# Chemical118/TREW

Hardware: AMD Instinct MI355X
Metric: Gbases/s scanned (short 5 32, 150 bp reads) (higher is better)
Workload: dtype u32

## Files before the change

### include/trew_hip.h

```cpp
#ifndef TREW_HIP_H
#define TREW_HIP_H

#include <stddef.h>
#include <stdint.h>

#ifdef __cplusplus
extern "C" {
#endif

#define TREW_HIP_ABI_VERSION 4

enum {
    TREW_MODE_SHORT = 0,
    TREW_MODE_PAIR = 1,
    TREW_MODE_LONG = 2,
    TREW_MODE_SEGMENT = 3
};

enum {
    TREW_TABLE_FORWARD_HIGH = 0,
    TREW_TABLE_FORWARD_LOW = 1,
    TREW_TABLE_BACKWARD_HIGH = 2,
    TREW_TABLE_BACKWARD_LOW = 3,
    TREW_TABLE_BOTH_HIGH = 4,
// ... 58 lines not shown
typedef struct {
    int32_t k;
    int32_t table;
    uint64_t word_lo;
    uint64_t word_hi;
    uint64_t count;
} trew_hip_row;

typedef struct trew_hip_ctx trew_hip_ctx;

int trew_hip_init(const trew_hip_params *params, trew_hip_ctx **out);
void trew_hip_destroy(trew_hip_ctx *ctx);
const char *trew_hip_last_error(const trew_hip_ctx *ctx);

int trew_hip_submit(trew_hip_ctx *ctx, const trew_hip_batch *batch, int slot);
int trew_hip_submit_ascii(trew_hip_ctx *ctx, const trew_hip_ascii_batch *batch, int slot);
int trew_hip_pack_ascii(trew_hip_ctx *ctx, const trew_hip_ascii_batch *batch, uint32_t *words, uint64_t words_cap, uint64_t *n_words);
int trew_hip_wait(trew_hip_ctx *ctx, int slot);

int trew_hip_collect(trew_hip_ctx *ctx, int table, trew_hip_row *rows, uint64_t cap, uint64_t *n_rows);
int trew_hip_reset_tables(trew_hip_ctx *ctx);
int trew_hip_add_rows(trew_hip_ctx *ctx, const trew_hip_row *rows, uint64_t n_rows);

int trew_hip_collect_device(trew_hip_ctx *ctx, trew_hip_row *d_rows, uint64_t cap, uint64_t *n_rows);
int trew_hip_add_rows_device(trew_hip_ctx *ctx, const trew_hip_row *d_rows, uint64_t n_rows);
int trew_hip_merge(trew_hip_ctx *dst, trew_hip_ctx *src);
int trew_hip_add_gathered_device(trew_hip_ctx *ctx, const trew_hip_row *d_buf, uint32_t n_slices, uint32_t own_slice,
                                 uint64_t slice_rows, void *producer_stream, uint64_t *max_rows);
int trew_hip_collect_slice_device(trew_hip_ctx *ctx, trew_hip_row *d_slice, uint64_t slice_rows, void *consumer_stream, uint64_t *n_rows);

int trew_hip_table_pressure(trew_hip_ctx *ctx, uint64_t *used_slots, uint64_t *total_slots, uint64_t *spilled_rows,
                            uint64_t *spill_capacity);

#define TREW_DEBUG_COUNTERS 8
int trew_hip_debug_counters(trew_hip_ctx *ctx, uint64_t *out, int n);

int trew_hip_debug_worklist(trew_hip_ctx *ctx, int slot, uint32_t *units, uint64_t cap, uint64_t *n);

int trew_hip_segment_results(trew_hip_ctx *ctx, int slot, int32_t *k_high, int32_t *k_low,
                             uint64_t *seq_high, uint64_t *seq_low, uint64_t *seq_high_hi, uint64_t *seq_low_hi,
                             uint64_t n_reads);
int trew_hip_filter_masks(trew_hip_ctx *ctx, const trew_hip_batch *batch, uint64_t *cand, int slots_per_read);

int trew_hip_last_timing(trew_hip_ctx *ctx, int slot, float *ms_filter, float *ms_exact, uint64_t *n_flagged);

typedef struct {
    int32_t k;
    int32_t reserved;
    uint64_t word;
} trew_hip_motif;
typedef struct {
    uint32_t windows_fwd, windows_rev, tract_start_fwd, tract_len_fwd, tract_start_rev, tract_len_rev;
} trew_hip_annot;
#define TREW_ANNOT_MAX_MOTIFS 8

int trew_motif_parse(const char *text, trew_hip_motif *out);
int trew_hip_annotate(trew_hip_ctx *ctx, const trew_hip_batch *batch, int slot, const trew_hip_motif *motifs, int n_motifs);
int trew_hip_annotate_results(trew_hip_ctx *ctx, int slot, trew_hip_annot *out, uint64_t cap, uint64_t *n, float *ms_kernel);
int trew_annotate_host(const uint32_t *words, const uint32_t *offsets, const uint32_t *lengths, uint64_t n_reads,
                       const trew_hip_motif *motifs, int n_motifs, trew_hip_annot *out);

typedef struct {
    uint32_t covered_fwd, head_len_fwd, head_cov_fwd, tail_len_fwd, tail_cov_fwd;
    uint32_t covered_rev, head_len_rev, head_cov_rev, tail_len_rev, tail_cov_rev;
} trew_hip_tract;
int trew_hip_tracts(trew_hip_ctx *ctx, const trew_hip_batch *batch, int slot, const trew_hip_motif *motifs, int n_motifs, int penalty);
int trew_hip_tracts_results(trew_hip_ctx *ctx, int slot, trew_hip_tract *out, uint64_t cap, uint64_t *n, float *ms_kernel);
// ... 61 lines not shown
```

### trew_amd/capi.py

```python
from __future__ import annotations

import ctypes as C
import os

import numpy as np

_HERE = os.path.dirname(os.path.abspath(__file__))
LIB_PATH = os.environ.get("TREW_HIP_LIB") or os.path.join(_HERE, "lib", "libtrew_hip.so")

MODE_SHORT, MODE_PAIR, MODE_LONG, MODE_SEGMENT = 0, 1, 2, 3
FLAG_NO_FILTER = 1
FLAG_DEBUG_POISON_LDS = 32
FLAG_NO_TIMING = 64
FLAG_COMPAT_G1 = 512
FLAG_TRACK_PRESSURE = 256
FLAG_DEBUG_NO_JOINT = 2048
FLAG_DEBUG_NO_UNI_DRAIN = 4096
FLAG_DEBUG_NO_GROUP = 1024
FLAG_DEBUG_ANNOT_GENERAL = 8192
FLAG_DEBUG_WIDE_NO_WAIT = 128
TABLE_NAMES = ("forward_high", "forward_low", "backward_high", "backward_low", "both_high", "both_low")

EXPORTED_SYMBOLS = (
    "trew_hip_init", "trew_hip_destroy", "trew_hip_last_error", "trew_hip_submit", "trew_hip_wait",
    "trew_hip_collect", "trew_hip_reset_tables", "trew_hip_add_rows", "trew_hip_segment_results",
    "trew_hip_filter_masks", "trew_hip_last_timing", "trew_pack_words", "trew_pack_reads",
    "trew_synth_short_ascii", "trew_synth_short_device", "trew_synth_pair_ascii", "trew_synth_pair_device",
    "trew_hip_malloc", "trew_hip_free", "trew_hip_memcpy_h2d", "trew_hip_memcpy_d2h", "trew_hip_abi_version",
    "trew_pack_pairs", "trew_hip_host_alloc", "trew_hip_host_free", "trew_hip_device_count",
    "trew_synth_long_lengths", "trew_synth_long_ascii", "trew_synth_long_device",
    "trew_hip_collect_device", "trew_hip_add_rows_device", "trew_hip_merge", "trew_hip_table_pressure",
    "trew_hip_add_gathered_device", "trew_hip_collect_slice_device", "trew_hip_debug_counters", "trew_hip_debug_worklist", "trew_hip_submit_ascii", "trew_hip_pack_ascii",
    "trew_motif_parse", "trew_hip_annotate", "trew_hip_annotate_results", "trew_annotate_host",
    "trew_hip_tracts", "trew_hip_tracts_results", "trew_tracts_host",
    "trew_hip_intervals", "trew_hip_intervals_results", "trew_intervals_host",
    "trew_hip_variants", "trew_hip_variants_results", "trew_variants_host",
)
DEBUG_COUNTERS = ("strict_rerun", "windows_fallback", "wide_spin_timeout", "inserted", "inserted_wide", "group_punt", "group_routed", "group_target")


class Params(C.Structure):
    _fields_ = [
        ("min_mer", C.c_int32), ("max_mer", C.c_int32),
        ("low_baseline", C.c_double), ("high_baseline", C.c_double),
        ("slice_length", C.c_int32), ("mode", C.c_int32), ("device", C.c_int32), ("n_slots", C.c_int32),
        ("max_batch_words", C.c_uint64), ("max_batch_reads", C.c_uint64),
        ("table_log2_slots", C.c_uint32), ("flags", C.c_uint32),
        ("max_batch_ascii_bytes", C.c_uint64),
    ]


class Batch(C.Structure):
    _fields_ = [
        ("words", C.c_void_p), ("n_words", C.c_uint64),
        ("offsets", C.c_void_p), ("lengths", C.c_void_p),
        ("uniform_length", C.c_uint32), ("uniform_stride", C.c_uint32),
        ("n_reads", C.c_uint64), ("on_device", C.c_int32), ("max_length", C.c_int32),
    ]


class AsciiBatch(C.Structure):
    _fields_ = [
        ("bases", C.c_void_p), ("n_bytes", C.c_uint64),
        ("byte_offsets", C.c_void_p), ("lengths", C.c_void_p), ("word_offsets", C.c_void_p),
        ("uniform_length", C.c_uint32), ("reserved", C.c_uint32), ("n_reads", C.c_uint64),
    ]


class Row(C.Structure):
    _fields_ = [("k", C.c_int32), ("table", C.c_int32), ("word_lo", C.c_uint64), ("word_hi", C.c_uint64),
                ("count", C.c_uint64)]
# ... 638 lines not shown
```

### trew_amd/csrc/kernels/prefilter.inc

```


__device__ __forceinline__ u32 xor_and(u32 x, u32 y, u32 m) { return __builtin_amdgcn_bitop3_b32(x, y, m, 0x28); }

__device__ __forceinline__ u64 all_k_mask(int kmin, int kmax) {
    if (kmax < kmin) return 0;
    u64 hi = kmax >= 64 ? ~0ull : ((1ull << kmax) - 1ull);
    u64 lo = (1ull << (kmin - 1)) - 1ull;
    return hi & ~lo;
}

template <int NW, int WS>
__device__ __forceinline__ u32 shr_word(const u32 (&x)[NW], int j, u32 bs) {
    const u32 lo = (j + WS < NW) ? x[j + WS < NW ? j + WS : 0] : 0u;
    const u32 hi = (j + WS + 1 < NW) ? x[j + WS + 1 < NW ? j + WS + 1 : 0] : 0u;
    return alignbit(hi, lo, bs);
}

template <int NW, int WS, int NWW>
__device__ __forceinline__ void filter_k(const u32 (&P1)[NW], const u32 (&P2)[NW], const u32 (&P3)[NW],
                                         const u32 (&v1)[NW], u32 (&V)[NW], int k, float lowf, u32 &cand_lo, u32 &cand_hi) {
    const u32 bs = (u32) k & 31u;
    u32 c01 = 0, c10 = 0, c11 = 0, count = 0;
#pragma unroll
    for (int j = 0; j < NWW; j++) {
// ... 281 lines not shown
            FilterRangeUni<NW, 2, NW, true>::run(P1, P2, P3, gmin > 64 ? gmin : 64, gmax, L, kmin, kmax, thr_row, dbg, vd);
        } else {
            FilterRangeUni<NW, 0, NW, false>::run(P1, P2, P3, gmin, g31, L, kmin, kmax, thr_row, false, vd);
            FilterRangeUni<NW, 1, NW, false>::run(P1, P2, P3, gmin > 32 ? gmin : 32, gmax < 63 ? gmax : 63, L, kmin, kmax, thr_row, false, vd);
            FilterRangeUni<NW, 2, NW, false>::run(P1, P2, P3, gmin > 64 ? gmin : 64, gmax, L, kmin, kmax, thr_row, false, vd);
            vd.flagm = vd.hasm;
        }
    }
}

struct HalvesP {
    u32 P1[3], P2[3];
};
__device__ __forceinline__ void halves_prefix(const u32 (&lo)[3], const u32 (&hi)[3], int L, HalvesP &o) {
    u32 none[3];
    segment_setup<3, false, false>(lo, hi,  lo, L,  none, o.P1, o.P2, none);
}
__device__ __forceinline__ u32 bcnt_acc_s(u32 x, int acc) {
    u32 d;
    asm("v_bcnt_u32_b32 %0, %1, %2" : "=v"(d) : "v"(x), "s"(acc));
    return d;
}
__device__ __forceinline__ void halves_signs(u32 F1a, u32 F2a, u32 F1b, u32 F2b, int n2, int n1, int K, u32 &x, u32 &t) {
    u32 a = bcnt_acc_s(F1a, n2);
    u32 b = bcnt_acc_s(F2a, n2);
    u32 c = bcnt_acc_s(F1a & F2a, n1);
    a = bcnt_acc(F1b, a);
    b = bcnt_acc(F2b, b);
    c = bcnt_acc(F1b & F2b, c);
    const u32 p = a - c, q = b - c;
    x = __builtin_amdgcn_bitop3_b32(p, q, c, 0x80);
    t = a + q + (u32) K;
}
__device__ __forceinline__ u64 halves_verdict(u32 xA, u32 tA, u32 xB, u32 tB) {
    const u32 y = __builtin_amdgcn_bitop3_b32(xA, xB, tA, 0x40);
    const u32 z = __builtin_amdgcn_bitop3_b32(y, tB, tB, 0x30);
    return __ballot((int) z >= 0);
}
struct Thr8 {
    int4 a, b;
};
__device__ __forceinline__ Thr8 load_thr8(const int4 *p) {
    typedef int v8i __attribute__((ext_vector_type(8)));
    typedef const __attribute__((address_space(4))) v8i *cptr;
    const v8i v = *(cptr) (unsigned long long) p;
    Thr8 o;
    o.a = make_int4(v[0], v[1], v[2], v[3]);
    o.b = make_int4(v[4], v[5], v[6], v[7]);
    return o;
}
__device__ __forceinline__ int4 load_thr4(const int4 *p) {
    typedef int v4i __attribute__((ext_vector_type(4)));
    typedef const __attribute__((address_space(4))) v4i *cptr;
    const v4i v = *(cptr) (unsigned long long) p;
    return make_int4(v.x, v.y, v.z, v.w);
}

__device__ __forceinline__ const int4 *joint_thresholds(const int2 *thr_tab) { return (const int4 *) (thr_tab + kThrRows * kThrRow); }

__device__ __forceinline__ u64 filter_halves_uni(const HalvesP &A, const HalvesP &Bh, int L, int klo, int khi, const int4 *__restrict__ thr_row,
                                                 const u32 *wm_tab) {
    u64 trig = 0;
    int k = klo;
    const int4 *tp = thr_row + (klo - 1);
    {
        int b = L - 64;
        b = b > khi ? khi : b;
        auto probe = [&](u32 bs, const int4 t) __attribute__((always_inline)) -> u64 {
            u32 xA, tA, xB, tB;
            halves_signs(A.P1[0] ^ alignbit(A.P1[1], A.P1[0], bs), A.P2[0] ^ alignbit(A.P2[1], A.P2[0], bs), A.P1[1] ^ alignbit(A.P1[2], A.P1[1], bs),
                         A.P2[1] ^ alignbit(A.P2[2], A.P2[1], bs), t.x, t.y, t.z, xA, tA);
            halves_signs(Bh.P1[0] ^ alignbit(Bh.P1[1], Bh.P1[0], bs), Bh.P2[0] ^ alignbit(Bh.P2[1], Bh.P2[0], bs), Bh.P1[1] ^ alignbit(Bh.P1[2], Bh.P1[1], bs),
                         Bh.P2[1] ^ alignbit(Bh.P2[2], Bh.P2[1], bs), t.x, t.y, t.z, xB, tB);
            return halves_verdict(xA, tA, xB, tB);
        };
        for (; k + 1 <= b; k += 2, tp += 2) {
            const Thr8 t8 = load_thr8(tp);
            trig |= probe((u32) k, t8.a);
            trig |= probe((u32) k + 1u, t8.b);
        }
        if (k <= b) {
            trig |= probe((u32) k, load_thr4(tp));
            k++, tp++;
        }
    }
    if (k <= khi) {
        const int b = khi;
        const int s = L > 63 ? L - 63 : 0;
        const u64 QA1 = container64(A.P1, s), QA2 = container64(A.P2, s), QB1 = container64(Bh.P1, s), QB2 = container64(Bh.P2, s);
        u32 sh = (u32) (k - s);
        typedef const __attribute__((address_space(3))) u32 *lds_u32;
        u32 wa = (u32) (unsigned long long) (lds_u32) wm_tab + 4u * (u32) (63 - (L - k));
        asm volatile("" : "+v"(wa));
        auto probe = [&](u32 shk, u32 wmk, const int4 t) __attribute__((always_inline)) -> u64 {
            const u64 SA1 = QA1 >> shk, SA2 = QA2 >> shk, SB1 = QB1 >> shk, SB2 = QB2 >> shk;
            const u32 gA1 = xor_and(A.P1[1], (u32) (SA1 >> 32), wmk), gA2 = xor_and(A.P2[1], (u32) (SA2 >> 32), wmk);
            const u32 gB1 = xor_and(Bh.P1[1], (u32) (SB1 >> 32), wmk), gB2 = xor_and(Bh.P2[1], (u32) (SB2 >> 32), wmk);
            u32 xA, tA, xB, tB;
            halves_signs(A.P1[0] ^ (u32) SA1, A.P2[0] ^ (u32) SA2, gA1, gA2, t.x, t.y, t.z, xA, tA);
            halves_signs(Bh.P1[0] ^ (u32) SB1, Bh.P2[0] ^ (u32) SB2, gB1, gB2, t.x, t.y, t.z, xB, tB);
            return halves_verdict(xA, tA, xB, tB);
        };
        for (; k + 1 <= b; k += 2, sh += 2u, wa += 8u, tp += 2) {
            const Thr8 t8 = load_thr8(tp);
            const u32 wm0 = *(lds_u32) (unsigned long long) wa, wm1 = *(lds_u32) (unsigned long long) (wa + 4u);
            trig |= probe(sh, wm0, t8.a);
            trig |= probe(sh + 1u, wm1, t8.b);
        }
        if (k <= b) trig |= probe(sh, *(lds_u32) (unsigned long long) wa, load_thr4(tp));
    }
    return trig;
}

constexpr int kCntThr = 97;
__device__ __forceinline__ int4 count_thresholds(int c, float lowf) {
    const float prod = __fmul_rn((float) c, lowf);
    const int ithr = (int) floorf(prod) + 1;
    return make_int4(-2 * ithr, -ithr, 4 * ithr - c - 1, ithr);
}

struct DrainHalf {
    u32 P1[3], P2[3], P3[3];
    u32 V[3];
};
__device__ __forceinline__ void drain_half_init(const u32 (&lo)[3], const u32 (&hi)[3], const u32 (&nm)[3], int L, bool active, DrainHalf &h) {
    segment_setup<3, false, true, true>(lo, hi, nm, L, h.V, h.P1, h.P2, h.P3);
#pragma unroll
    for (int j = 0; j < 3; j++) h.V[j] = active ? h.V[j] : 0u;
}
__device__ __forceinline__ void drain_v_step3(u32 (&V)[3]) {
    V[0] &= alignbit(V[1], V[0], 1u);
    V[1] &= alignbit(V[2], V[1], 1u);
    V[2] &= V[2] >> 1;
}
template <int N>
__device__ __forceinline__ int drain_signs(const u32 (&F1)[N], const u32 (&F2)[N], const int4 th) {
    u32 a = (u32) th.x, b = (u32) th.x, c = (u32) th.y;
#pragma unroll
    for (int j = 0; j < N; j++) {
        a = bcnt_acc(F1[j], a);
        b = bcnt_acc(F2[j], b);
        c = bcnt_acc(F1[j] & F2[j], c);
    }
    const u32 p = a - c, q = b - c;
    const u32 t = a + q + (u32) th.z;
    return (int) __builtin_amdgcn_bitop3_b32(__builtin_amdgcn_bitop3_b32(p, q, c, 0x80), t, t, 0x30);
}
template <int N>
__device__ __forceinline__ bool drain_pass8(const u32 (&F1)[N], const u32 (&F2)[N], const u32 (&F3)[N], const u32 (&V)[N], u32 count, int ithr) {
    const u32 m8 = max_bucket8<N>(F1, F2, F3, V, count);
    return (int) m8 >= ithr;
}

__device__ __forceinline__ bool drain_uni_applies(const DevParams &P, u32 UL, int gmax_run) {
    const int n_halves = P.mode == TREW_MODE_PAIR ? 4 : (P.mode == TREW_MODE_SHORT ? 2 : 0);
    if (n_halves == 0) return false;
    for (int slot = n_halves; slot < mode_slots(P.mode); slot++)
        if (get_segment(P.mode, slot, UL, UL, P.min_mer, P.max_mer, P.slice_len).valid) return false;
    for (int p = 0; p < n_halves; p += 2) {
        const Segment a = get_segment(P.mode, p, UL, UL, P.min_mer, P.max_mer, P.slice_len);
        const Segment b = get_segment(P.mode, p + 1, UL, UL, P.min_mer, P.max_mer, P.slice_len);
        const int la = (int) a.len, lb = (int) b.len, lmin = la < lb ? la : lb, lmax = la < lb ? lb : la;
        const int khi = a.kmax < gmax_run ? a.kmax : gmax_run;
        if (!(a.valid && b.valid && a.kmin == b.kmin && a.kmax == b.kmax && lmax <= 95 && lmax - lmin <= 1 && a.kmin >= 1 && khi <= lmin)) return false;
    }
    return true;
}

__device__ __forceinline__ bool filter_deferred_uni(const DevParams &P, const DevBatch &B, u64 unit, bool active, int gmax_run,
                                                    const int4 *cnt_thr) {
    const u32 UL = B.uniform_length;
    ReadRef rd[2];
    unit_reads(P, B, unit, active, rd);
    const u64 actm = __ballot(active);
    u64 flag = 0;
    const int n_halves = P.mode == TREW_MODE_PAIR ? 4 : 2;
    for (int p = 0; p < n_halves && flag != actm; p += 2) {
        const Segment sA = get_segment(P.mode, p, UL, UL, P.min_mer, P.max_mer, P.slice_len);
        const Segment sB = get_segment(P.mode, p + 1, UL, UL, P.min_mer, P.max_mer, P.slice_len);
        const int LA = rfl_i((int) sA.len), LB = rfl_i((int) sB.len), Lmax = LA < LB ? LB : LA;
        const int klo = rfl_i(sA.kmin > P.min_mer ? sA.kmin : P.min_mer), khi = rfl_i(sA.kmax < gmax_run ? sA.kmax : gmax_run);
        DrainHalf A, Bh;
        {
            u32 lo[3], hi[3], nm[3];
            load_planes<3>(sA.mate ? rd[1] : rd[0], sA.start, lo, hi, nm);
            drain_half_init(lo, hi, nm, LA, active, A);
            load_planes<3>(sB.mate ? rd[1] : rd[0], sB.start, lo, hi, nm);
            drain_half_init(lo, hi, nm, LB, active, Bh);
        }
        for (int t = 1; t < klo; t++) {
            drain_v_step3(A.V);
            drain_v_step3(Bh.V);
        }
        int k = klo;
        {
            const int b = khi < Lmax - 64 ? khi : Lmax - 64;
            auto half3 = [&](const DrainHalf &h, u32 bs) __attribute__((always_inline)) -> u64 {
                const u32 cnt = bcnt_acc(h.V[2], bcnt_acc(h.V[1], __popc(h.V[0])));
                const int4 th = cnt_thr[cnt];
                u32 F1[3], F2[3];
#pragma unroll
                for (int j = 0; j < 3; j++) {
                    F1[j] = xor_and(h.P1[j], alignbit(j < 2 ? h.P1[j < 2 ? j + 1 : 0] : 0u, h.P1[j], bs), h.V[j]);
                    F2[j] = xor_and(h.P2[j], alignbit(j < 2 ? h.P2[j < 2 ? j + 1 : 0] : 0u, h.P2[j], bs), h.V[j]);
                }
                const u64 p4 = __ballot(drain_signs<3>(F1, F2, th) >= 0);
                u64 p8 = 0;
                if (p4 & ~flag) {
                    u32 F3[3];
#pragma unroll
                    for (int j = 0; j < 3; j++) F3[j] = h.P3[j] ^ alignbit(j < 2 ? h.P3[j < 2 ? j + 1 : 0] : 0u, h.P3[j], bs);
                    p8 = __ballot(drain_pass8<3>(F1, F2, F3, h.V, cnt, th.w));
                }
                return p8;
            };
            for (; k <= b && flag != actm; k++) {
                flag |= half3(A, (u32) k);
                flag |= half3(Bh, (u32) k);
                drain_v_step3(A.V);
                drain_v_step3(Bh.V);
            }
        }
        if (k <= khi && flag != actm) {
            const int oA = LA > 63 ? LA - 63 : 0, oB = LB > 63 ? LB - 63 : 0;
            const u64 QA1 = container64(A.P1, oA), QA2 = container64(A.P2, oA), QB1 = container64(Bh.P1, oB), QB2 = container64(Bh.P2, oB);
            u64 VA = ((u64) A.V[1] << 32) | A.V[0], VB = ((u64) Bh.V[1] << 32) | Bh.V[0];
            auto half2 = [&](const DrainHalf &h, u64 Q1, u64 Q2, u64 V, int s) __attribute__((always_inline)) -> u64 {
                const u32 v0 = (u32) V, v1 = (u32) (V >> 32);
                const u32 cnt = bcnt_acc(v1, __popc(v0));
                const int4 th = cnt_thr[cnt];
                const u32 sh = (u32) (k - s);
                const u64 S1 = Q1 >> sh, S2 = Q2 >> sh;
                const u32 F1[2] = {xor_and(h.P1[0], (u32) S1, v0), xor_and(h.P1[1], (u32) (S1 >> 32), v1)};
                const u32 F2[2] = {xor_and(h.P2[0], (u32) S2, v0), xor_and(h.P2[1], (u32) (S2 >> 32), v1)};
                const u64 p4 = __ballot(drain_signs<2>(F1, F2, th) >= 0);
                u64 p8 = 0;
                if (p4 & ~flag) {
                    const u64 S3 = container64(h.P3, s) >> sh;
                    const u32 F3[2] = {h.P3[0] ^ (u32) S3, h.P3[1] ^ (u32) (S3 >> 32)};
                    const u32 Vw[2] = {v0, v1};
                    p8 = __ballot(drain_pass8<2>(F1, F2, F3, Vw, cnt, th.w));
                }
                return p8;
            };
            for (; k <= khi && flag != actm; k++) {
                flag |= half2(A, QA1, QA2, VA, oA);
                flag |= half2(Bh, QB1, QB2, VB, oB);
                VA &= VA >> 1;
                VB &= VB >> 1;
            }
        }
    }
    return (flag >> lane_id()) & 1ull;
}

constexpr u32 kFilterThreads = TREW_FILTER_THREADS;
constexpr u32 kStage = kFilterThreads == 256 ? 1024 : 192;
constexpr u32 kDefer = 2 * kFilterThreads;

template <int NW>
#ifndef TREW_FILTER3_WAVES
#define TREW_FILTER3_WAVES 6
#endif
#ifndef TREW_FILTER5_WAVES
#define TREW_FILTER5_WAVES 6
#endif
__global__ __launch_bounds__(kFilterThreads, (NW <= 3 ? TREW_FILTER3_WAVES : (NW == 5 ? TREW_FILTER5_WAVES : 1))) void filter_kernel(DevParams P, DevBatch B, u32 *wl, u32 *wl_count, u32 wl_cap,
                                                                u64 *dbg_masks, int dbg_slots, int max_seg, u32 *diag,
                                                                const int2 *__restrict__ thr_tab) {
#ifdef TREW_AB_FILTER_PRIO
    __builtin_amdgcn_s_setprio(TREW_AB_FILTER_PRIO);
#endif
    __shared__ u32 stage[kStage];
    __shared__ u32 stage_n, flush_base;
    __shared__ u32 defer_n;
    u32 defer_seen = 0;
    if (threadIdx.x == 0) stage_n = 0;
    __syncthreads();
    auto flush = [&]() __attribute__((always_inline)) {
        const u32 n = stage_n;
        if (n) {
            if (threadIdx.x == 0) flush_base = atomicAdd(wl_count, n);
            __syncthreads();
            const u32 fb = flush_base;
            for (u32 i = threadIdx.x; i < n; i += blockDim.x) {
                if (fb + i < wl_cap)
                    wl[fb + i] = stage[i];
                else
                    atomicAdd(&diag[kDiagWorklistDrop], 1u);
            }
            __syncthreads();
            if (threadIdx.x == 0) stage_n = 0;
        }
        __syncthreads();
    };
    auto append = [&](bool flag, u32 unit) __attribute__((always_inline)) {
        wave_append(&stage_n, flag, [&](u32 at) __attribute__((always_inline)) { stage[at] = unit; });
        __syncthreads();
        const bool full = stage_n > kStage - kFilterThreads;
        defer_seen = defer_n;
        __syncthreads();
        if (full) flush();
    };
    const int nslots = mode_slots(P.mode);
    const int gmax_run = (P.flags & TREW_FLAG_DEBUG_NO_KLOOP) ? P.min_mer - 1 : P.max_mer;
    auto general = [&](u64 unit, bool active) __attribute__((always_inline)) -> u64 {
        ReadRef rd[2];
        unit_reads(P, B, unit, active, rd);
        u64 any = 0;
#pragma unroll
        for (int slot = 0; slot < kMaxSlots; slot++) {
            if (slot < nslots) {
                u64 mask = 0;
                Segment sg = get_segment(P.mode, slot, rd[0].len, rd[1].len, P.min_mer, P.max_mer, P.slice_len);
                const bool ok = active && sg.valid && sg.len <= (u32) (32 * NW - 1);
                if (__any(ok)) {
                    u32 lo[NW], hi[NW], nm[NW];
                    const ReadRef &r = sg.mate ? rd[1] : rd[0];
                    if (ok) {
                        load_planes<NW>(r, sg.start, lo, hi, nm);
                    } else {
#pragma unroll
                        for (int j = 0; j < NW; j++) {
                            lo[j] = hi[j] = 0;
                            nm[j] = 0xffffffffu;
                        }
                    }
                    u64 m;
                    if (P.flags & TREW_FLAG_NO_FILTER)
                        m = all_k_mask(sg.kmin, sg.kmax);
                    else
                        m = filter_segment<NW>(lo, hi, nm, ok ? (int) sg.len : 0, sg.kmin, sg.kmax, P.min_mer, gmax_run, max_seg, P.lowf);
                    mask = ok ? m : 0ull;
                }
                if (active && sg.valid && sg.len > (u32) (32 * NW - 1)) mask = all_k_mask(sg.kmin, sg.kmax);
                any |= mask;
                if (dbg_masks && active && slot < dbg_slots) dbg_masks[unit * (u64) dbg_slots + slot] = mask;
            }
        }
        return any;
    };

    __shared__ u32 defer[kDefer];
    __shared__ unsigned char defer_kind[kDefer];
    __shared__ u32 wm_tab[34];
    if (threadIdx.x < 34) wm_tab[threadIdx.x] = threadIdx.x < 32 ? 0xffffffffu >> threadIdx.x : 0u;
    __shared__ int4 cnt_thr[kCntThr];
    for (u32 i = threadIdx.x; i < (u32) kCntThr; i += blockDim.x) cnt_thr[i] = count_thresholds((int) i, P.lowf);
    const u32 UL = B.uniform_length;
    const bool uni = NW <= 5 && UL != 0 && thr_tab != nullptr && P.mode != TREW_MODE_LONG && !(P.flags & TREW_FLAG_NO_FILTER);
    const bool uni_drain = NW == 3 && uni && !dbg_masks && !(P.flags & TREW_FLAG_DEBUG_NO_UNI_DRAIN) && drain_uni_applies(P, UL, gmax_run);
    if (threadIdx.x == 0) defer_n = 0;
    __syncthreads();
    __shared__ u32 next_chunk[2];
    constexpr u32 kChunkShards = 8;
    const u32 my_shard = blockIdx.x & (kChunkShards - 1u);
    auto shard_ctr = [&](u32 sh) __attribute__((always_inline)) { return wl_count + 32u + 32u * sh + kChunkCounterWord; };
    u64 chunk = blockIdx.x;
    u32 round = 0;
    for (;;) {
        const bool more = chunk * kFilterThreads < B.n_units;
        if (more) {
            const u64 unit = chunk * kFilterThreads + threadIdx.x;
            const bool active = unit < B.n_units;
            u32 nxt = 0;
            if (threadIdx.x == 0) nxt = gridDim.x + kChunkShards * atomicAdd(shard_ctr(my_shard), 1u) + my_shard;
            u64 any = 0;
            bool dfr = active, dfr_n = false;
            if constexpr (NW <= 5) {
                if (uni) {
                    ReadRef rd[2];
                    unit_reads(P, B, unit, active, rd);
                    dfr = false;
                    int slot0 = 0;
                    if constexpr (NW == 3) {
                        const int n_halves = P.mode == TREW_MODE_PAIR ? 4 : (P.mode == TREW_MODE_SHORT ? 2 : 0);
                        for (; slot0 + 1 < n_halves && !dbg_masks && !(P.flags & TREW_FLAG_DEBUG_NO_JOINT); slot0 += 2) {
                            const Segment sA = get_segment(P.mode, slot0, UL, UL, P.min_mer, P.max_mer, P.slice_len);
                            const Segment sB = get_segment(P.mode, slot0 + 1, UL, UL, P.min_mer, P.max_mer, P.slice_len);
                            const int L = rfl_i((int) sA.len);
                            const int klo = rfl_i(sA.kmin > P.min_mer ? sA.kmin : P.min_mer), khi = rfl_i(sA.kmax < gmax_run ? sA.kmax : gmax_run);
                            const bool uneq = sB.len == sA.len + 1u;
                            if (!(sA.valid && sB.valid && (sA.len == sB.len || uneq) && sA.len <= 95u && sA.kmin == sB.kmin && sA.kmax == sB.kmax &&
                                  klo >= L + 1 - kUniSubsetMax && khi <= L - 32 && klo <= 31))
                                break;
                            u32 loA[3], hiA[3], nmA[3], loB[3], hiB[3], nmB[3];
                            load_planes<3>(sA.mate ? rd[1] : rd[0], sA.start, loA, hiA, nmA);
                            load_planes<3>(sB.mate ? rd[1] : rd[0], sB.start, loB, hiB, nmB);
                            const u32 anyn = segment_has_n<3>(nmA, L) | segment_has_n<3>(nmB, (int) sB.len);
                            dfr = dfr || (active && anyn != 0);
                            dfr_n = dfr_n || (active && anyn != 0);
                            HalvesP hA, hB;
                            halves_prefix(loA, hiA, L, hA);
                            halves_prefix(loB, hiB, L, hB);
                            const u64 trig = filter_halves_uni(hA, hB, L, klo, khi, joint_thresholds(thr_tab) + (uneq ? 2 + slot0 / 2 : slot0 / 2) * kThrRow, wm_tab);
                            dfr = dfr || (active && any == 0 && ((trig >> lane_id()) & 1ull) != 0);
                        }
                    }
                    for (int slot = slot0; slot < nslots; slot++) {
                        const Segment sg = get_segment(P.mode, slot, UL, UL, P.min_mer, P.max_mer, P.slice_len);
                        if (!sg.valid) continue;
                        if (sg.len > (u32) (32 * NW - 1)) {
                            dfr = dfr || active;
                            continue;
                        }
                        u32 lo[NW], hi[NW], nm[NW];
                        const ReadRef r = sg.mate ? rd[1] : rd[0];
                        load_planes<NW>(r, sg.start, lo, hi, nm);
                        u32 anyn = 0;
#pragma unroll
                        for (int j = 0; j < NW; j++) {
                            const int bits = (int) sg.len - 32 * j;
                            const u32 lm = low_mask(bits);
                            anyn |= nm[j] & lm;
                        }
                        UniVerdict vd;
                        filter_segment_uni<NW>(lo, hi, (int) sg.len, sg.kmin, sg.kmax, P.min_mer, gmax_run, thr_tab + slot * kThrRow, dbg_masks != nullptr, vd);
                        dfr = dfr || (active && anyn != 0);
                        dfr_n = dfr_n || (active && anyn != 0);
                        any |= (vd.flagm >> lane_id()) & 1ull;
                        if (dbg_masks && active && anyn == 0 && slot < dbg_slots)
                            dbg_masks[unit * (u64) dbg_slots + slot] = ((((u64) vd.chi) << 32) | vd.clo) & all_k_mask(sg.kmin, sg.kmax);
                    }
                }
            }
            {
                wave_append(&defer_n, dfr, [=](u32 at) __attribute__((always_inline)) {
                    defer[at] = (u32) unit;
                    defer_kind[at] = dfr_n ? 1 : 0;
                });
            }
            if (threadIdx.x == 0) next_chunk[round & 1u] = nxt;
            append(active && !dfr && any != 0, (u32) unit);
            chunk = next_chunk[round & 1u];
            if (chunk * kFilterThreads >= B.n_units) {
                __syncthreads();
                if (threadIdx.x == 0) {
                    u64 c = chunk;
                    for (u32 att = 1; att < kChunkShards && c * kFilterThreads >= B.n_units; att++) {
                        const u32 sh = (my_shard + att) & (kChunkShards - 1u);
                        c = (u64) gridDim.x + (u64) kChunkShards * atomicAdd(shard_ctr(sh), 1u) + sh;
                    }
                    next_chunk[round & 1u] = (u32) (c < 0xffffffffull ? c : 0xffffffffull);
                }
                __syncthreads();
                chunk = next_chunk[round & 1u];
                __syncthreads();
            }
            round++;
        }
        const u32 dn = defer_seen;
        if (dn >= kFilterThreads || (!more && dn > 0u)) {
            const u32 take = dn < kFilterThreads ? dn : kFilterThreads;
            const u32 at = dn - take;
            const bool active2 = threadIdx.x < take;
            const u32 unit2 = active2 ? defer[at + threadIdx.x] : 0u;
            const bool n2 = active2 && defer_kind[at + threadIdx.x] != 0;
            __syncthreads();
            if (threadIdx.x == 0) defer_n = at;
#ifndef TREW_AB_SKIP_DRAIN
            const u64 any2 = uni_drain ? (u64) filter_deferred_uni(P, B, unit2, active2, gmax_run, cnt_thr) : general(unit2, active2);
#else
            u64 any2 = 0;
            u32 keep = unit2;
            asm volatile("" : "+v"(keep), "+v"(any2));
            (void) keep;
#endif
            append(active2 && any2 != 0 && !n2, unit2);
            append(active2 && any2 != 0 && n2, unit2);
        } else if (!more) {
            break;
        }
    }
    flush();
}
```

### trew_amd/csrc/trew_capi.cpp

```cpp
#include <hip/hip_runtime.h>

#include <algorithm>
#include <atomic>
#include <cmath>
#include <cstdio>
#include <cstdlib>
#include <cstring>
#include <mutex>
#include <string>
#include <thread>
#include <vector>

#include "trew_common.hpp"
#include "trew_launch.hpp"
#include "trew_measures_host.hpp"
#include "trew_synth.hpp"

using namespace trew;

namespace {

enum Measure { kAnnotate, kTracts, kIntervals, kVariants, kMeasures };
const char *const kMeasureName[kMeasures] = {"annotate", "tracts", "intervals", "variants"};
struct DevBuf {
// ... 941 lines not shown
    HIPCHK(ctx, hipMemsetAsync(ctx->d_row_flags, 0, kRowFlagWords * 4, st));
    HIPCHK(ctx, launch_add_gathered(st, ctx->table, d_buf, n_slices, own_slice, slice_rows, ctx->d_row_flags));
    u32 flags[kRowFlagWords] = {0, 0, 0, 0};
    HIPCHK(ctx, hipMemcpyAsync(flags, ctx->d_row_flags, sizeof(flags), hipMemcpyDeviceToHost, st));
    HIPCHK(ctx, hipStreamSynchronize(st));
    if (max_rows) *max_rows = ((u64) flags[kRowFlagMaxHi] << 32) | flags[kRowFlagMaxLo];
    if (flags[kRowFlagBad]) return fail(ctx, "trew_hip_add_gathered_device: row out of range (nothing was added)");
    if (flags[kRowFlagOverflow]) return 0;
    u32 diag[kDiagWords];
    return check_diag(ctx, diag);
}

extern "C" int trew_hip_debug_worklist(trew_hip_ctx *ctx, int slot, uint32_t *units, uint64_t cap, uint64_t *n) {
    if (!ctx || !n) return -1;
    if (slot < 0 || slot >= (int) ctx->slots.size()) return fail(ctx, "slot out of range");
    HIPCHK(ctx, hipSetDevice(ctx->p.device));
    Slot &s = ctx->slots[(size_t) slot];
    HIPCHK(ctx, hipStreamSynchronize(s.stream));
    u32 c = 0;
    if (s.n_launches) HIPCHK(ctx, hipMemcpy(&c, s.d_wl_count + ((s.n_launches - 1) & 1) * kWlCountWords, 4, hipMemcpyDeviceToHost));
    c = (u32) std::min<u64>(c, ctx->p.max_batch_reads);
    *n = c;
    const u64 take = std::min<u64>(c, cap);
    if (units && take) HIPCHK(ctx, hipMemcpy(units, s.d_wl, take * 4, hipMemcpyDeviceToHost));
    return 0;
}

extern "C" int trew_hip_debug_counters(trew_hip_ctx *ctx, uint64_t *out, int n) {
    if (!ctx || !out || n < 0) return -1;
    if (int rc = sync_all(ctx)) return rc;
    u32 diag[kDiagWords], fb[kFallbackWords];
    HIPCHK(ctx, hipMemcpy(diag, ctx->table.overflow, sizeof(diag), hipMemcpyDeviceToHost));
    HIPCHK(ctx, fallback_counters_read(fb));
    const u32 v[TREW_DEBUG_COUNTERS] = {fb[kFallbackStrictRerun], fb[kFallbackWindows], fb[kFallbackWideSpin], diag[kDiagInserted], diag[kDiagInsertedWide], fb[kFallbackGroupPunt], fb[kFallbackGroupRouted], fb[kFallbackGroupTarget]};
    for (int i = 0; i < n; i++) out[i] = i < TREW_DEBUG_COUNTERS ? v[i] : 0;
    return 0;
}

extern "C" int trew_hip_merge(trew_hip_ctx *dst, trew_hip_ctx *src) {
    if (!dst || !src) return -1;
    if (dst == src) return fail(dst, "trew_hip_merge: source and destination are the same context");
    std::mutex *m1 = &dst->table_mu, *m2 = &src->table_mu;
    if (m2 < m1) std::swap(m1, m2);
    std::lock_guard<std::mutex> l1(*m1), l2(*m2);
    if (int rc = sync_all(src)) return rc;
    u64 n = 0;
    if (int rc = compact_to(src, -1, nullptr, 0, &n)) return rc;
    if (n == 0) return 0;
    if (int rc = ensure_rows(src, &src->d_collect_rows, &src->collect_cap, n)) return rc;
    if (int rc = compact_to(src, -1, src->d_collect_rows, src->collect_cap, &n)) return rc;
    if (int rc = sync_all(dst)) return rc;
    if (int rc = ensure_rows(dst, &dst->d_add_rows, &dst->add_cap, n)) return rc;
    HIPCHK(dst, hipSetDevice(dst->p.device));
    HIPCHK(dst, hipMemcpyPeerAsync(dst->d_add_rows, dst->p.device, src->d_collect_rows, src->p.device, n * sizeof(trew_hip_row), dst->slots[0].stream));
    return add_device_rows_locked(dst, dst->d_add_rows, n, false);
}

extern "C" int trew_hip_segment_results(trew_hip_ctx *ctx, int slot, int32_t *k_high, int32_t *k_low,
                                        uint64_t *seq_high, uint64_t *seq_low, uint64_t *seq_high_hi, uint64_t *seq_low_hi,
                                        uint64_t n_reads) {
    if (!ctx) return -1;
    if (ctx->p.mode != TREW_MODE_SEGMENT) return fail(ctx, "segment results exist only in TREW_MODE_SEGMENT");
    if (slot < 0 || slot >= (int) ctx->slots.size()) return fail(ctx, "slot out of range");
    if (int rc = trew_hip_wait(ctx, slot)) return rc;
    Slot &s = ctx->slots[(size_t) slot];
    if (n_reads > s.n_units) return fail(ctx, "n_reads exceeds the last batch");
    if (k_high) HIPCHK(ctx, hipMemcpy(k_high, s.res.k_high, n_reads * 4, hipMemcpyDeviceToHost));
// ... 615 lines not shown
```

### trew_amd/csrc/trew_common.hpp

```cpp
#pragma once
#include <stdint.h>

#include "../../include/trew_hip.h"

namespace trew {

typedef uint32_t u32;
typedef uint64_t u64;

constexpr int kMaxSlots = 6;
constexpr int kMaxSegBases = 1023;
constexpr int kTablePartBits = 9;
constexpr int kThrRows = kMaxSlots + 2;
constexpr int kThrJointRows = 4;
constexpr int kThrRow = 66;
constexpr size_t kThrTableBytes = (size_t) kThrRows * kThrRow * 8 + (size_t) kThrJointRows * kThrRow * 16;
constexpr int kThrNever = 1 << 20;

struct DevParams {
    int min_mer, max_mer;
    double low, high;
    float lowf;
    int slice_len;
    int mode;
// ... 1 lines not shown
};

struct DevBatch {
    const u32 *words;
    const u32 *offsets;
    const u32 *lengths;
    u32 uniform_length;
    u32 uniform_stride;
    u64 n_reads;
    u64 n_units;
};

constexpr int kChunkCounterWord = 16;

enum {
    kDiagOverflow = 0,
    kDiagWorklistDrop = 1,
    kDiagIntentDrop = 2,
    kDiagInserted = 3,
    kDiagInsertedWide = 4,
    kDiagKernarg = 5,
    kDiagSpillRows = 6,
    kDiagG1Drop = 7,
    kDiagWords = 16
};

enum {
    kFallbackStrictRerun = 0,
    kFallbackWindows = 1,
    kFallbackWideSpin = 2,
    kFallbackGroupPunt = 3,
    kFallbackGroupRouted = 4,
    kFallbackGroupTarget = 5,
    kFallbackWords = 8
};

enum { kRowFlagBad = 0, kRowFlagOverflow = 1, kRowFlagMaxLo = 2, kRowFlagMaxHi = 3, kRowFlagWords = 4 };

struct DevTable {
    u64 *keys;
    u64 *counts;
    u32 log2_part_slots;
    u32 *overflow;
    const struct DevWide *wide;
};

struct DevG1 {
    trew_hip_row *log;
    u32 *counters;
    unsigned char *pair_flags;
    u32 log_cap;
};


struct DevWide {
    u64 *wtag, *wlo, *whi, *wcount;
    u32 wide_log2_slots;
    u32 spill_cap;
    trew_hip_row *spill_rows;
    u32 *spill_n;
    u32 spin_limit;
};

struct DevTableG1 {
    DevTable t;
    DevG1 g;
// ... 143 lines not shown
```

Measured before the change: 1996.

## Drain only the single flagged half when one read half passes the joint filter

The joint halves prefilter now keeps a separate pass verdict for each half instead of a combined ballot. When exactly one half of a unit needs exact checking, the unit goes to a new per-half defer list and a single-half drain that processes only that half's planes. This avoids running the two-half drain on halves the filter already rejected. The cost is an extra shared-memory defer queue, extra wave appends and an added debug atomic counter on every drain.

Result: faster. 2090 (median of 6 runs) (+4.7%).

```diff
diff --git a/include/trew_hip.h b/include/trew_hip.h
--- a/include/trew_hip.h
+++ b/include/trew_hip.h
@@ -114,7 +114,7 @@
 int trew_hip_table_pressure(trew_hip_ctx *ctx, uint64_t *used_slots, uint64_t *total_slots, uint64_t *spilled_rows,
                             uint64_t *spill_capacity);
 
-#define TREW_DEBUG_COUNTERS 8
+#define TREW_DEBUG_COUNTERS 10
 int trew_hip_debug_counters(trew_hip_ctx *ctx, uint64_t *out, int n);
 
 int trew_hip_debug_worklist(trew_hip_ctx *ctx, int slot, uint32_t *units, uint64_t cap, uint64_t *n);
diff --git a/trew_amd/capi.py b/trew_amd/capi.py
--- a/trew_amd/capi.py
+++ b/trew_amd/capi.py
@@ -36,7 +36,8 @@
     "trew_hip_intervals", "trew_hip_intervals_results", "trew_intervals_host",
     "trew_hip_variants", "trew_hip_variants_results", "trew_variants_host",
 )
-DEBUG_COUNTERS = ("strict_rerun", "windows_fallback", "wide_spin_timeout", "inserted", "inserted_wide", "group_punt", "group_routed", "group_target")
+DEBUG_COUNTERS = ("strict_rerun", "windows_fallback", "wide_spin_timeout", "inserted", "inserted_wide", "group_punt", "group_routed", "group_target",
+                  "half_drain", "unit_drain")
 
 
 class Params(C.Structure):
diff --git a/trew_amd/csrc/kernels/prefilter.inc b/trew_amd/csrc/kernels/prefilter.inc
--- a/trew_amd/csrc/kernels/prefilter.inc
+++ b/trew_amd/csrc/kernels/prefilter.inc
@@ -337,11 +337,7 @@
     x = __builtin_amdgcn_bitop3_b32(p, q, c, 0x80);
     t = a + q + (u32) K;
 }
-__device__ __forceinline__ u64 halves_verdict(u32 xA, u32 tA, u32 xB, u32 tB) {
-    const u32 y = __builtin_amdgcn_bitop3_b32(xA, xB, tA, 0x40);
-    const u32 z = __builtin_amdgcn_bitop3_b32(y, tB, tB, 0x30);
-    return __ballot((int) z >= 0);
-}
+__device__ __forceinline__ u32 halves_note(u32 acc, u32 x, u32 t) { return __builtin_amdgcn_bitop3_b32(acc, x, t, 0x40); }
 struct Thr8 {
     int4 a, b;
 };
@@ -363,29 +359,30 @@
 
 __device__ __forceinline__ const int4 *joint_thresholds(const int2 *thr_tab) { return (const int4 *) (thr_tab + kThrRows * kThrRow); }
 
-__device__ __forceinline__ u64 filter_halves_uni(const HalvesP &A, const HalvesP &Bh, int L, int klo, int khi, const int4 *__restrict__ thr_row,
-                                                 const u32 *wm_tab) {
-    u64 trig = 0;
+__device__ __forceinline__ void filter_halves_uni(const HalvesP &A, const HalvesP &Bh, int L, int klo, int khi, const int4 *__restrict__ thr_row,
+                                                  const u32 *wm_tab, bool &passA, bool &passB) {
+    u32 accA = 0xffffffffu, accB = 0xffffffffu;
     int k = klo;
     const int4 *tp = thr_row + (klo - 1);
     {
         int b = L - 64;
         b = b > khi ? khi : b;
-        auto probe = [&](u32 bs, const int4 t) __attribute__((always_inline)) -> u64 {
+        auto probe = [&](u32 bs, const int4 t) __attribute__((always_inline)) {
             u32 xA, tA, xB, tB;
             halves_signs(A.P1[0] ^ alignbit(A.P1[1], A.P1[0], bs), A.P2[0] ^ alignbit(A.P2[1], A.P2[0], bs), A.P1[1] ^ alignbit(A.P1[2], A.P1[1], bs),
                          A.P2[1] ^ alignbit(A.P2[2], A.P2[1], bs), t.x, t.y, t.z, xA, tA);
             halves_signs(Bh.P1[0] ^ alignbit(Bh.P1[1], Bh.P1[0], bs), Bh.P2[0] ^ alignbit(Bh.P2[1], Bh.P2[0], bs), Bh.P1[1] ^ alignbit(Bh.P1[2], Bh.P1[1], bs),
                          Bh.P2[1] ^ alignbit(Bh.P2[2], Bh.P2[1], bs), t.x, t.y, t.z, xB, tB);
-            return halves_verdict(xA, tA, xB, tB);
+            accA = halves_note(accA, xA, tA);
+            accB = halves_note(accB, xB, tB);
         };
         for (; k + 1 <= b; k += 2, tp += 2) {
             const Thr8 t8 = load_thr8(tp);
-            trig |= probe((u32) k, t8.a);
-            trig |= probe((u32) k + 1u, t8.b);
+            probe((u32) k, t8.a);
+            probe((u32) k + 1u, t8.b);
         }
         if (k <= b) {
-            trig |= probe((u32) k, load_thr4(tp));
+            probe((u32) k, load_thr4(tp));
             k++, tp++;
         }
     }
@@ -397,24 +394,26 @@
         typedef const __attribute__((address_space(3))) u32 *lds_u32;
         u32 wa = (u32) (unsigned long long) (lds_u32) wm_tab + 4u * (u32) (63 - (L - k));
         asm volatile("" : "+v"(wa));
-        auto probe = [&](u32 shk, u32 wmk, const int4 t) __attribute__((always_inline)) -> u64 {
+        auto probe = [&](u32 shk, u32 wmk, const int4 t) __attribute__((always_inline)) {
             const u64 SA1 = QA1 >> shk, SA2 = QA2 >> shk, SB1 = QB1 >> shk, SB2 = QB2 >> shk;
             const u32 gA1 = xor_and(A.P1[1], (u32) (SA1 >> 32), wmk), gA2 = xor_and(A.P2[1], (u32) (SA2 >> 32), wmk);
             const u32 gB1 = xor_and(Bh.P1[1], (u32) (SB1 >> 32), wmk), gB2 = xor_and(Bh.P2[1], (u32) (SB2 >> 32), wmk);
             u32 xA, tA, xB, tB;
             halves_signs(A.P1[0] ^ (u32) SA1, A.P2[0] ^ (u32) SA2, gA1, gA2, t.x, t.y, t.z, xA, tA);
             halves_signs(Bh.P1[0] ^ (u32) SB1, Bh.P2[0] ^ (u32) SB2, gB1, gB2, t.x, t.y, t.z, xB, tB);
-            return halves_verdict(xA, tA, xB, tB);
+            accA = halves_note(accA, xA, tA);
+            accB = halves_note(accB, xB, tB);
         };
         for (; k + 1 <= b; k += 2, sh += 2u, wa += 8u, tp += 2) {
             const Thr8 t8 = load_thr8(tp);
             const u32 wm0 = *(lds_u32) (unsigned long long) wa, wm1 = *(lds_u32) (unsigned long long) (wa + 4u);
-            trig |= probe(sh, wm0, t8.a);
-            trig |= probe(sh + 1u, wm1, t8.b);
-        }
-        if (k <= b) trig |= probe(sh, *(lds_u32) (unsigned long long) wa, load_thr4(tp));
-    }
-    return trig;
+            probe(sh, wm0, t8.a);
+            probe(sh + 1u, wm1, t8.b);
+        }
+        if (k <= b) probe(sh, *(lds_u32) (unsigned long long) wa, load_thr4(tp));
+    }
+    passA = (int) accA >= 0;
+    passB = (int) accB >= 0;
 }
 
 constexpr int kCntThr = 97;
@@ -462,14 +461,54 @@
     if (n_halves == 0) return false;
     for (int slot = n_halves; slot < mode_slots(P.mode); slot++)
         if (get_segment(P.mode, slot, UL, UL, P.min_mer, P.max_mer, P.slice_len).valid) return false;
+    const Segment first = get_segment(P.mode, 0, UL, UL, P.min_mer, P.max_mer, P.slice_len);
     for (int p = 0; p < n_halves; p += 2) {
         const Segment a = get_segment(P.mode, p, UL, UL, P.min_mer, P.max_mer, P.slice_len);
         const Segment b = get_segment(P.mode, p + 1, UL, UL, P.min_mer, P.max_mer, P.slice_len);
         const int la = (int) a.len, lb = (int) b.len, lmin = la < lb ? la : lb, lmax = la < lb ? lb : la;
         const int khi = a.kmax < gmax_run ? a.kmax : gmax_run;
         if (!(a.valid && b.valid && a.kmin == b.kmin && a.kmax == b.kmax && lmax <= 95 && lmax - lmin <= 1 && a.kmin >= 1 && khi <= lmin)) return false;
+        if (a.kmin != first.kmin || a.kmax != first.kmax) return false;
     }
     return true;
+}
+
+__device__ __forceinline__ u64 drain_probe3(const DrainHalf &h, u32 bs, u64 flag, const int4 *cnt_thr) {
+    const u32 cnt = bcnt_acc(h.V[2], bcnt_acc(h.V[1], __popc(h.V[0])));
+    const int4 th = cnt_thr[cnt];
+    u32 F1[3], F2[3];
+#pragma unroll
+    for (int j = 0; j < 3; j++) {
+        F1[j] = xor_and(h.P1[j], alignbit(j < 2 ? h.P1[j < 2 ? j + 1 : 0] : 0u, h.P1[j], bs), h.V[j]);
+        F2[j] = xor_and(h.P2[j], alignbit(j < 2 ? h.P2[j < 2 ? j + 1 : 0] : 0u, h.P2[j], bs), h.V[j]);
+    }
+    const u64 p4 = __ballot(drain_signs<3>(F1, F2, th) >= 0);
+    u64 p8 = 0;
+    if (p4 & ~flag) {
+        u32 F3[3];
+#pragma unroll
+        for (int j = 0; j < 3; j++) F3[j] = h.P3[j] ^ alignbit(j < 2 ? h.P3[j < 2 ? j + 1 : 0] : 0u, h.P3[j], bs);
+        p8 = __ballot(drain_pass8<3>(F1, F2, F3, h.V, cnt, th.w));
+    }
+    return p8;
+}
+__device__ __forceinline__ u64 drain_probe2(const DrainHalf &h, u64 Q1, u64 Q2, u64 V, int s, int k, u64 flag, const int4 *cnt_thr) {
+    const u32 v0 = (u32) V, v1 = (u32) (V >> 32);
+    const u32 cnt = bcnt_acc(v1, __popc(v0));
+    const int4 th = cnt_thr[cnt];
+    const u32 sh = (u32) (k - s);
+    const u64 S1 = Q1 >> sh, S2 = Q2 >> sh;
+    const u32 F1[2] = {xor_and(h.P1[0], (u32) S1, v0), xor_and(h.P1[1], (u32) (S1 >> 32), v1)};
+    const u32 F2[2] = {xor_and(h.P2[0], (u32) S2, v0), xor_and(h.P2[1], (u32) (S2 >> 32), v1)};
+    const u64 p4 = __ballot(drain_signs<2>(F1, F2, th) >= 0);
+    u64 p8 = 0;
+    if (p4 & ~flag) {
+        const u64 S3 = container64(h.P3, s) >> sh;
+        const u32 F3[2] = {h.P3[0] ^ (u32) S3, h.P3[1] ^ (u32) (S3 >> 32)};
+        const u32 Vw[2] = {v0, v1};
+        p8 = __ballot(drain_pass8<2>(F1, F2, F3, Vw, cnt, th.w));
+    }
+    return p8;
 }
 
 __device__ __forceinline__ bool filter_deferred_uni(const DevParams &P, const DevBatch &B, u64 unit, bool active, int gmax_run,
@@ -498,62 +537,68 @@
             drain_v_step3(Bh.V);
         }
         int k = klo;
-        {
-            const int b = khi < Lmax - 64 ? khi : Lmax - 64;
-            auto half3 = [&](const DrainHalf &h, u32 bs) __attribute__((always_inline)) -> u64 {
-                const u32 cnt = bcnt_acc(h.V[2], bcnt_acc(h.V[1], __popc(h.V[0])));
-                const int4 th = cnt_thr[cnt];
-                u32 F1[3], F2[3];
-#pragma unroll
-                for (int j = 0; j < 3; j++) {
-                    F1[j] = xor_and(h.P1[j], alignbit(j < 2 ? h.P1[j < 2 ? j + 1 : 0] : 0u, h.P1[j], bs), h.V[j]);
-                    F2[j] = xor_and(h.P2[j], alignbit(j < 2 ? h.P2[j < 2 ? j + 1 : 0] : 0u, h.P2[j], bs), h.V[j]);
-                }
-                const u64 p4 = __ballot(drain_signs<3>(F1, F2, th) >= 0);
-                u64 p8 = 0;
-                if (p4 & ~flag) {
-                    u32 F3[3];
-#pragma unroll
-                    for (int j = 0; j < 3; j++) F3[j] = h.P3[j] ^ alignbit(j < 2 ? h.P3[j < 2 ? j + 1 : 0] : 0u, h.P3[j], bs);
-                    p8 = __ballot(drain_pass8<3>(F1, F2, F3, h.V, cnt, th.w));
-                }
-                return p8;
-            };
-            for (; k <= b && flag != actm; k++) {
-                flag |= half3(A, (u32) k);
-                flag |= half3(Bh, (u32) k);
-                drain_v_step3(A.V);
-                drain_v_step3(Bh.V);
-            }
+        for (const int b = khi < Lmax - 64 ? khi : Lmax - 64; k <= b && flag != actm; k++) {
+            flag |= drain_probe3(A, (u32) k, flag, cnt_thr);
+            flag |= drain_probe3(Bh, (u32) k, flag, cnt_thr);
+            drain_v_step3(A.V);
+            drain_v_step3(Bh.V);
         }
         if (k <= khi && flag != actm) {
             const int oA = LA > 63 ? LA - 63 : 0, oB = LB > 63 ? LB - 63 : 0;
             const u64 QA1 = container64(A.P1, oA), QA2 = container64(A.P2, oA), QB1 = container64(Bh.P1, oB), QB2 = container64(Bh.P2, oB);
             u64 VA = ((u64) A.V[1] << 32) | A.V[0], VB = ((u64) Bh.V[1] << 32) | Bh.V[0];
-            auto half2 = [&](const DrainHalf &h, u64 Q1, u64 Q2, u64 V, int s) __attribute__((always_inline)) -> u64 {
-                const u32 v0 = (u32) V, v1 = (u32) (V >> 32);
-                const u32 cnt = bcnt_acc(v1, __popc(v0));
-                const int4 th = cnt_thr[cnt];
-                const u32 sh = (u32) (k - s);
-                const u64 S1 = Q1 >> sh, S2 = Q2 >> sh;
-                const u32 F1[2] = {xor_and(h.P1[0], (u32) S1, v0), xor_and(h.P1[1], (u32) (S1 >> 32), v1)};
-                const u32 F2[2] = {xor_and(h.P2[0], (u32) S2, v0), xor_and(h.P2[1], (u32) (S2 >> 32), v1)};
-                const u64 p4 = __ballot(drain_signs<2>(F1, F2, th) >= 0);
-                u64 p8 = 0;
-                if (p4 & ~flag) {
-                    const u64 S3 = container64(h.P3, s) >> sh;
-                    const u32 F3[2] = {h.P3[0] ^ (u32) S3, h.P3[1] ^ (u32) (S3 >> 32)};
-                    const u32 Vw[2] = {v0, v1};
-                    p8 = __ballot(drain_pass8<2>(F1, F2, F3, Vw, cnt, th.w));
-                }
-                return p8;
-            };
             for (; k <= khi && flag != actm; k++) {
-                flag |= half2(A, QA1, QA2, VA, oA);
-                flag |= half2(Bh, QB1, QB2, VB, oB);
+                flag |= drain_probe2(A, QA1, QA2, VA, oA, k, flag, cnt_thr);
+                flag |= drain_probe2(Bh, QB1, QB2, VB, oB, k, flag, cnt_thr);
                 VA &= VA >> 1;
                 VB &= VB >> 1;
             }
+        }
+    }
+    return (flag >> lane_id()) & 1ull;
+}
+
+__device__ __forceinline__ bool filter_deferred_half(const DevParams &P, const DevBatch &B, u64 unit, u32 half, bool active, int gmax_run,
+                                                     const int4 *cnt_thr) {
+    const u32 UL = B.uniform_length;
+    ReadRef rd[2];
+    unit_reads(P, B, unit, active, rd);
+    Segment sg = get_segment(P.mode, 0, UL, UL, P.min_mer, P.max_mer, P.slice_len);
+    int Lmax = (int) sg.len;
+    const int n_halves = P.mode == TREW_MODE_PAIR ? 4 : 2;
+    for (int slot = 1; slot < n_halves; slot++) {
+        const Segment o = get_segment(P.mode, slot, UL, UL, P.min_mer, P.max_mer, P.slice_len);
+        Lmax = (int) o.len > Lmax ? (int) o.len : Lmax;
+        if (half == (u32) slot) {
+            sg.mate = o.mate;
+            sg.start = o.start;
+            sg.len = o.len;
+        }
+    }
+    Lmax = rfl_i(Lmax);
+    const int L = (int) sg.len;
+    const int klo = rfl_i(sg.kmin > P.min_mer ? sg.kmin : P.min_mer), khi = rfl_i(sg.kmax < gmax_run ? sg.kmax : gmax_run);
+    DrainHalf h;
+    {
+        u32 lo[3], hi[3], nm[3];
+        load_planes<3>(sg.mate ? rd[1] : rd[0], sg.start, lo, hi, nm);
+        drain_half_init(lo, hi, nm, L, active, h);
+    }
+    for (int t = 1; t < klo; t++) drain_v_step3(h.V);
+    const u64 actm = __ballot(active);
+    u64 flag = 0;
+    int k = klo;
+    for (const int b = khi < Lmax - 64 ? khi : Lmax - 64; k <= b && flag != actm; k++) {
+        flag |= drain_probe3(h, (u32) k, flag, cnt_thr);
+        drain_v_step3(h.V);
+    }
+    if (k <= khi && flag != actm) {
+        const int o = L > 63 ? L - 63 : 0;
+        const u64 Q1 = container64(h.P1, o), Q2 = container64(h.P2, o);
+        u64 V = ((u64) h.V[1] << 32) | h.V[0];
+        for (; k <= khi && flag != actm; k++) {
+            flag |= drain_probe2(h, Q1, Q2, V, o, k, flag, cnt_thr);
+            V &= V >> 1;
         }
     }
     return (flag >> lane_id()) & 1ull;
@@ -578,8 +623,8 @@
 #endif
     __shared__ u32 stage[kStage];
     __shared__ u32 stage_n, flush_base;
-    __shared__ u32 defer_n;
-    u32 defer_seen = 0;
+    __shared__ u32 defer_n, half_n;
+    u32 defer_seen = 0, half_seen = 0;
     if (threadIdx.x == 0) stage_n = 0;
     __syncthreads();
     auto flush = [&]() __attribute__((always_inline)) {
@@ -604,6 +649,7 @@
         __syncthreads();
         const bool full = stage_n > kStage - kFilterThreads;
         defer_seen = defer_n;
+        if constexpr (NW == 3) half_seen = half_n;
         __syncthreads();
         if (full) flush();
     };
@@ -648,6 +694,9 @@
 
     __shared__ u32 defer[kDefer];
     __shared__ unsigned char defer_kind[kDefer];
+    constexpr u32 kHalfDefer = NW == 3 ? kDefer : 1;
+    __shared__ u32 hdefer[kHalfDefer];
+    __shared__ unsigned char hdefer_kind[kHalfDefer];
     __shared__ u32 wm_tab[34];
     if (threadIdx.x < 34) wm_tab[threadIdx.x] = threadIdx.x < 32 ? 0xffffffffu >> threadIdx.x : 0u;
     __shared__ int4 cnt_thr[kCntThr];
@@ -656,6 +705,9 @@
     const bool uni = NW <= 5 && UL != 0 && thr_tab != nullptr && P.mode != TREW_MODE_LONG && !(P.flags & TREW_FLAG_NO_FILTER);
     const bool uni_drain = NW == 3 && uni && !dbg_masks && !(P.flags & TREW_FLAG_DEBUG_NO_UNI_DRAIN) && drain_uni_applies(P, UL, gmax_run);
     if (threadIdx.x == 0) defer_n = 0;
+    if constexpr (NW == 3) {
+        if (threadIdx.x == 0) half_n = 0;
+    }
     __syncthreads();
     __shared__ u32 next_chunk[2];
     constexpr u32 kChunkShards = 8;
@@ -672,6 +724,8 @@
             if (threadIdx.x == 0) nxt = gridDim.x + kChunkShards * atomicAdd(shard_ctr(my_shard), 1u) + my_shard;
             u64 any = 0;
             bool dfr = active, dfr_n = false;
+            bool dfr_half = false;
+            u32 hsel = 0;
             if constexpr (NW <= 5) {
                 if (uni) {
                     ReadRef rd[2];
@@ -680,6 +734,7 @@
                     int slot0 = 0;
                     if constexpr (NW == 3) {
                         const int n_halves = P.mode == TREW_MODE_PAIR ? 4 : (P.mode == TREW_MODE_SHORT ? 2 : 0);
+                        u32 nneed = 0;
                         for (; slot0 + 1 < n_halves && !dbg_masks && !(P.flags & TREW_FLAG_DEBUG_NO_JOINT); slot0 += 2) {
                             const Segment sA = get_segment(P.mode, slot0, UL, UL, P.min_mer, P.max_mer, P.slice_len);
                             const Segment sB = get_segment(P.mode, slot0 + 1, UL, UL, P.min_mer, P.max_mer, P.slice_len);
@@ -692,15 +747,19 @@
                             u32 loA[3], hiA[3], nmA[3], loB[3], hiB[3], nmB[3];
                             load_planes<3>(sA.mate ? rd[1] : rd[0], sA.start, loA, hiA, nmA);
                             load_planes<3>(sB.mate ? rd[1] : rd[0], sB.start, loB, hiB, nmB);
-                            const u32 anyn = segment_has_n<3>(nmA, L) | segment_has_n<3>(nmB, (int) sB.len);
-                            dfr = dfr || (active && anyn != 0);
-                            dfr_n = dfr_n || (active && anyn != 0);
+                            const u32 nA = segment_has_n<3>(nmA, L), nB = segment_has_n<3>(nmB, (int) sB.len);
+                            dfr_n = dfr_n || (active && (nA | nB) != 0);
                             HalvesP hA, hB;
                             halves_prefix(loA, hiA, L, hA);
                             halves_prefix(loB, hiB, L, hB);
-                            const u64 trig = filter_halves_uni(hA, hB, L, klo, khi, joint_thresholds(thr_tab) + (uneq ? 2 + slot0 / 2 : slot0 / 2) * kThrRow, wm_tab);
-                            dfr = dfr || (active && any == 0 && ((trig >> lane_id()) & 1ull) != 0);
+                            bool passA, passB;
+                            filter_halves_uni(hA, hB, L, klo, khi, joint_thresholds(thr_tab) + (uneq ? 2 + slot0 / 2 : slot0 / 2) * kThrRow, wm_tab, passA, passB);
+                            const bool needA = active && (nA != 0 || passA), needB = active && (nB != 0 || passB);
+                            nneed += (u32) needA + (u32) needB;
+                            hsel = needB ? (u32) slot0 + 1u : (needA ? (u32) slot0 : hsel);
+                            dfr = dfr || needA || needB;
                         }
+                        dfr_half = uni_drain && slot0 == n_halves && nneed == 1u;
                     }
                     for (int slot = slot0; slot < nslots; slot++) {
                         const Segment sg = get_segment(P.mode, slot, UL, UL, P.min_mer, P.max_mer, P.slice_len);
@@ -730,9 +789,13 @@
                 }
             }
             {
-                wave_append(&defer_n, dfr, [=](u32 at) __attribute__((always_inline)) {
+                wave_append(&defer_n, dfr && !dfr_half, [=](u32 at) __attribute__((always_inline)) {
                     defer[at] = (u32) unit;
                     defer_kind[at] = dfr_n ? 1 : 0;
+                });
+                if constexpr (NW == 3) wave_append(&half_n, dfr_half, [=](u32 at) __attribute__((always_inline)) {
+                    hdefer[at] = (u32) unit;
+                    hdefer_kind[at] = (unsigned char) ((hsel << 1) | (dfr_n ? 1u : 0u));
                 });
             }
             if (threadIdx.x == 0) next_chunk[round & 1u] = nxt;
@@ -754,25 +817,38 @@
             }
             round++;
         }
-        const u32 dn = defer_seen;
-        if (dn >= kFilterThreads || (!more && dn > 0u)) {
-            const u32 take = dn < kFilterThreads ? dn : kFilterThreads;
-            const u32 at = dn - take;
+        const u32 dn = defer_seen, hn = half_seen;
+        auto drain = [&](const u32 *list, const unsigned char *kind, u32 *list_n, u32 n, bool halves) __attribute__((always_inline)) {
+            const u32 take = n < kFilterThreads ? n : kFilterThreads;
+            const u32 at = n - take;
             const bool active2 = threadIdx.x < take;
-            const u32 unit2 = active2 ? defer[at + threadIdx.x] : 0u;
-            const bool n2 = active2 && defer_kind[at + threadIdx.x] != 0;
+            const u32 unit2 = active2 ? list[at + threadIdx.x] : 0u;
+            const u32 kind2 = active2 ? kind[at + threadIdx.x] : 0u;
+            const bool n2 = (kind2 & 1u) != 0;
             __syncthreads();
-            if (threadIdx.x == 0) defer_n = at;
+            if (threadIdx.x == 0) {
+                *list_n = at;
+                if (halves || uni_drain) atomicAdd(&g_fallback[halves ? kFallbackHalfDrain : kFallbackUnitDrain], take);
+            }
 #ifndef TREW_AB_SKIP_DRAIN
-            const u64 any2 = uni_drain ? (u64) filter_deferred_uni(P, B, unit2, active2, gmax_run, cnt_thr) : general(unit2, active2);
+            const u64 any2 = halves      ? (u64) filter_deferred_half(P, B, unit2, kind2 >> 1, active2, gmax_run, cnt_thr)
+                             : uni_drain ? (u64) filter_deferred_uni(P, B, unit2, active2, gmax_run, cnt_thr)
+                                         : general(unit2, active2);
 #else
             u64 any2 = 0;
-            u32 keep = unit2;
+            u32 keep = unit2 + kind2;
             asm volatile("" : "+v"(keep), "+v"(any2));
             (void) keep;
 #endif
             append(active2 && any2 != 0 && !n2, unit2);
             append(active2 && any2 != 0 && n2, unit2);
+        };
+        const bool drain_units = dn >= kFilterThreads || (!more && dn > 0u), drain_halves = NW == 3 && (hn >= kFilterThreads || (!more && hn > 0u));
+        if (drain_units || drain_halves) {
+            if (drain_units) drain(defer, defer_kind, &defer_n, dn, false);
+            if constexpr (NW == 3) {
+                if (drain_halves) drain(hdefer, hdefer_kind, &half_n, hn, true);
+            }
         } else if (!more) {
             break;
         }
diff --git a/trew_amd/csrc/trew_capi.cpp b/trew_amd/csrc/trew_capi.cpp
--- a/trew_amd/csrc/trew_capi.cpp
+++ b/trew_amd/csrc/trew_capi.cpp
@@ -997,7 +997,7 @@
     u32 diag[kDiagWords], fb[kFallbackWords];
     HIPCHK(ctx, hipMemcpy(diag, ctx->table.overflow, sizeof(diag), hipMemcpyDeviceToHost));
     HIPCHK(ctx, fallback_counters_read(fb));
-    const u32 v[TREW_DEBUG_COUNTERS] = {fb[kFallbackStrictRerun], fb[kFallbackWindows], fb[kFallbackWideSpin], diag[kDiagInserted], diag[kDiagInsertedWide], fb[kFallbackGroupPunt], fb[kFallbackGroupRouted], fb[kFallbackGroupTarget]};
+    const u32 v[TREW_DEBUG_COUNTERS] = {fb[kFallbackStrictRerun], fb[kFallbackWindows], fb[kFallbackWideSpin], diag[kDiagInserted], diag[kDiagInsertedWide], fb[kFallbackGroupPunt], fb[kFallbackGroupRouted], fb[kFallbackGroupTarget], fb[kFallbackHalfDrain], fb[kFallbackUnitDrain]};
     for (int i = 0; i < n; i++) out[i] = i < TREW_DEBUG_COUNTERS ? v[i] : 0;
     return 0;
 }
diff --git a/trew_amd/csrc/trew_common.hpp b/trew_amd/csrc/trew_common.hpp
--- a/trew_amd/csrc/trew_common.hpp
+++ b/trew_amd/csrc/trew_common.hpp
@@ -57,6 +57,8 @@
     kFallbackGroupPunt = 3,
     kFallbackGroupRouted = 4,
     kFallbackGroupTarget = 5,
+    kFallbackHalfDrain = 6,
+    kFallbackUnitDrain = 7,
     kFallbackWords = 8
 };
 
```
